# cyberfabric/cyberfabric-core

Hardware: NVIDIA H100
Metric: prompt_bytes_per_sec_bpe_encode (higher is better)
Workload: dtype u32

## Files before the change

### cyberfabric-core_b200/csrc/bpe_kernels.cuh

```cuda
#pragma once
#include <stdint.h>

#include "pretok.cuh"
#include "pretok_fsm.h"
#include "pretok_sync.cuh"
#include "tables.h"
#include "tma.cuh"

namespace cfbpe {

#ifdef CUSIM_EMULATOR
#define CFBPE_DYN_SMEM(name) uint32_t* const name = reinterpret_cast<uint32_t*>(cusim::dyn_smem())
#else
#define CFBPE_DYN_SMEM(name) extern __shared__ __align__(16) uint32_t name[]
#endif

constexpr uint32_t kMaxVocabs = 8;
#ifdef CUSIM_EMULATOR
inline unsigned long long* dbg_counters() { static unsigned long long c[16]; return c; }
#define CFBPE_DBG_COUNT(i) (++dbg_counters()[i])
#else
#define CFBPE_DBG_COUNT(i) ((void)0)
#endif

#ifndef CFBPE_SPLIT_CHUNK
#define CFBPE_SPLIT_CHUNK 64
#endif
constexpr uint32_t kSplitChunk = CFBPE_SPLIT_CHUNK;
constexpr uint32_t kBigPiece = 256;
constexpr uint32_t kScanTileWords = 256;

struct VocabSet {
    TablesView v[kMaxVocabs];
    uint32_t loaded_mask;
};

struct BatchView {
    const uint8_t* bytes;
    const uint64_t* offsets;
    const uint8_t* vocab_ids;
    uint32_t n_prompts;
    uint64_t total_bytes;
};

struct DeviceStatus {
    uint32_t bad_utf8;
    uint32_t n_long;
    uint32_t long_overflow;
    uint32_t long_next;
    uint32_t n_big;
    uint32_t defer_next;
    uint64_t n_tokens;
    uint64_t tok_end;
    unsigned long long long_bytes;
    unsigned long long long_tokens;
    uint32_t miss_n[3];
    uint32_t miss_next[3];
    uint32_t miss_overflow;
    uint32_t extra_n;
    uint32_t split_next;
    uint32_t fix_n;
    uint32_t bad_vocab;
    uint32_t defer_n;
    unsigned long long defer_parts;
};

struct MissLists {
    uint64_t* list[3];
    uint32_t cap[3];
};
__host__ __device__ inline uint32_t miss_class_min_len(uint32_t c) { return c == 0 ? 13u : (c == 1 ? 7u : 1u); }

struct LongPiece { uint64_t start; uint64_t end; uint32_t vocab; uint32_t pad; };

__device__ __forceinline__ uint32_t find_prompt(const uint64_t* __restrict__ offsets, uint32_t n, uint64_t pos) {
    uint32_t lo = 0, hi = n;
    while (hi - lo > 1) {
        const uint32_t mid = (lo + hi) >> 1;
        if (offsets[mid] <= pos) lo = mid; else hi = mid;
    }
    return lo;
}

__device__ __forceinline__ void or_bits(uint32_t* __restrict__ words, uint64_t word, uint32_t bits) {
    if (bits) atomicOr(&words[word], bits);
}

__device__ __forceinline__ void prefetch_l2(const void* p) {
#if !defined(CUSIM_EMULATOR)
    asm volatile("prefetch.global.L2 [%0];" ::"l"(p));
#else
    (void)p;
#endif
}

__device__ __forceinline__ uint64_t same_byte_run_end(const uint8_t* __restrict__ s, uint64_t pos, uint64_t pe, uint32_t c) {
    uint64_t e = pos;
    while (e < pe && (reinterpret_cast<uintptr_t>(s + e) & 15u)) { if (s[e] != c) return e; ++e; }
    const uint32_t w = c * 0x01010101u;
    for (uint64_t a = e; a < pe && a < e + 1024; a += 128) prefetch_l2(s + a);
    while (e + 128 <= pe) {
        if (e + 1024 < pe) prefetch_l2(s + e + 1024);
        uint4 v[8];
#pragma unroll
        for (uint32_t k = 0; k < 8; ++k) v[k] = *reinterpret_cast<const uint4*>(s + e + 16 * k);
        uint32_t d = 0;
#pragma unroll
        for (uint32_t k = 0; k < 8; ++k) d |= (v[k].x ^ w) | (v[k].y ^ w) | (v[k].z ^ w) | (v[k].w ^ w);
        if (d) break;
        e += 128;
    }
    while (e + 16 <= pe) {
        const uint4 v = *reinterpret_cast<const uint4*>(s + e);
        if (v.x != w || v.y != w || v.z != w || v.w != w) break;
        e += 16;
    }
    while (e < pe && s[e] == c) ++e;
    return e;
}
__device__ __forceinline__ bool four_ascii_digits(uint32_t w) {
    const uint32_t t = w ^ 0x30303030u;
    return ((((t & 0x7F7F7F7Fu) + 0x76767676u) | t) & 0x80808080u) == 0u;
}
__device__ __forceinline__ uint64_t ascii_digit_run_end(const uint8_t* __restrict__ s, uint64_t pos, uint64_t pe) {
    uint64_t e = pos;
    while (e < pe && (reinterpret_cast<uintptr_t>(s + e) & 15u)) { if ((s[e] - '0') >= 10u) return e; ++e; }
// ... 322 lines not shown
        sid[bi * 32] = best;
        const uint32_t above2 = alive & ~((2u << bi) - 1u);
        const uint32_t below = alive & ((1u << bi) - 1u);
        const bool wr = above2 != 0, wl = below != 0;
        const uint32_t nn = wr ? static_cast<uint32_t>(__ffs(above2)) - 1u : 0u;
        const uint32_t pv = wl ? 31u - static_cast<uint32_t>(__clz(below)) : 0u;
        uint32_t nr, nl;
        pair_lookup2(T, best, wr ? sid[nn * 32] : 0u, wr, wl ? sid[pv * 32] : 0u, best, wl, nr, nl);
        srk[bi * 32] = nr == kNone ? kNone : ((nr << 5) | bi);
        if (wl) srk[pv * 32] = nl == kNone ? kNone : ((nl << 5) | pv);
    }
    const uint64_t mask = static_cast<uint64_t>(alive) << (pos & 31);
    atomicOr(&tok_bits[pos >> 5], static_cast<uint32_t>(mask));
    if (mask >> 32) atomicOr(&tok_bits[(pos >> 5) + 1], static_cast<uint32_t>(mask >> 32));
    return alive;
}

__device__ __forceinline__ uint32_t kth_set_bit(uint32_t mask, uint32_t k) {
    for (uint32_t i = 0; i < k; ++i) mask &= mask - 1;
    return __ffs(mask) - 1;
}

constexpr uint32_t kPieceMulti = 0x80000000u;
constexpr uint32_t kPieceLong = 0xFFFFFFFEu;
constexpr uint32_t kPieceTileBytes = kPieceWarps * kPieceRange;
static_assert(kPieceTileBytes == 64 * 32, "K3 derives a word's piece tile as word >> 6");
struct DenseIds {
    uint32_t* by_piece;
    uint32_t* extras;
    uint32_t extras_cap;
    uint32_t* tile_pieces;
    uint64_t* piece_base;
};

__global__ void __launch_bounds__(kPieceWarps * 32)
long_scan_kernel(BatchView b, const uint32_t* __restrict__ piece_bits, LongPiece* __restrict__ long_list, uint32_t long_cap,
                 DeviceStatus* status, uint32_t* __restrict__ tile_pieces) {
    const uint32_t lane = threadIdx.x & 31, wic = threadIdx.x >> 5;
    const uint64_t warp = static_cast<uint64_t>(blockIdx.x) * kPieceWarps + wic;
    const uint64_t r0 = warp * kPieceRange;
    const uint64_t r1 = (r0 + kPieceRange < b.total_bytes) ? r0 + kPieceRange : b.total_bytes;
    const bool multi = b.vocab_ids != nullptr;
    const uint64_t base = r0 + 16ull * lane;
    const uint32_t my = (base < b.total_bytes) ? ((piece_bits[base >> 5] >> (16u * (lane & 1u))) & 0xFFFFu) : 0u;
    uint32_t v = my ? (16u * lane + static_cast<uint32_t>(__ffs(my)) - 1u) : 0xFFFFu;
#pragma unroll
    for (uint32_t d = 1; d < 32; d <<= 1) { const uint32_t o = __shfl_down_sync(kFull, v, d); if (lane + d < 32 && o < v) v = o; }
    uint32_t nf_rel = __shfl_down_sync(kFull, v, 1);
    if (lane == 31) nf_rel = 0xFFFFu;
    const bool any_open = __any_sync(kFull, my != 0 && nf_rel == 0xFFFFu);
    uint64_t beyond = b.total_bytes;
    if (any_open) beyond = next_set_bit(piece_bits, r1, b.total_bytes);
    const uint64_t nf = (nf_rel == 0xFFFFu) ? beyond : r0 + nf_rel;
    __shared__ uint32_t s_n[2], s_at[2], s_pieces;
    __shared__ unsigned long long s_bytes;
    if (threadIdx.x < 2) s_n[threadIdx.x] = 0;
    if (threadIdx.x == 0) { s_bytes = 0; s_pieces = 0; }
    __syncthreads();
    const uint32_t np = __reduce_add_sync(kFull, static_cast<uint32_t>(__popc(my)));
    if (lane == 0 && np) atomicAdd(&s_pieces, np);
    bool is_long = false, big = false;
    uint32_t k = 0, pv = 0;
    uint64_t pos = 0;
    if (my && r0 < b.total_bytes) {
        pos = base + (31u - static_cast<uint32_t>(__clz(my)));
        if (nf - pos > 32) {
            is_long = true;
            big = (nf - pos) > kBigPiece;
            pv = multi ? b.vocab_ids[find_prompt(b.offsets, b.n_prompts, pos)] : 0u;
            k = atomicAdd(&s_n[big ? 1 : 0], 1u);
            atomicAdd(&s_bytes, static_cast<unsigned long long>(nf - pos));
        }
    }
    __syncthreads();
    if (threadIdx.x < 2 && s_n[threadIdx.x]) s_at[threadIdx.x] = atomicAdd(threadIdx.x ? &status->n_big : &status->n_long, s_n[threadIdx.x]);
    if (threadIdx.x == 2 && s_bytes) atomicAdd(&status->long_bytes, s_bytes);
    if (threadIdx.x == 3) tile_pieces[blockIdx.x] = s_pieces;
    __syncthreads();
    if (is_long) {
        const uint32_t idx = s_at[big ? 1 : 0] + k;
        if (idx < long_cap) { LongPiece lp; lp.start = pos; lp.end = nf; lp.vocab = pv; lp.pad = 0; long_list[big ? long_cap - 1 - idx : idx] = lp; }
        else atomicOr(&status->long_overflow, 1u);
    }
}

constexpr uint32_t kLookupWarps = 4;
static_assert(kLookupWarps == kPieceWarps, "K2a's CTA is the 2 KiB tile K2s counted");
__global__ void __launch_bounds__(kLookupWarps * 32)
bpe_lookup_kernel(BatchView b, VocabSet vs, const uint32_t* __restrict__ piece_bits, DenseIds dn, MissLists ml, DeviceStatus* status) {
    __shared__ uint16_t s_pos[kLookupWarps][kPieceRange + 2];
    __shared__ uint64_t s_miss0[kLookupWarps * kPieceRange / 13 + 8];
    __shared__ uint64_t s_miss1[kLookupWarps * kPieceRange / 7 + 8];
    __shared__ uint64_t s_miss2[kLookupWarps * kPieceRange / 2 + 8];
    __shared__ uint32_t s_cnt[3], s_base[3], s_nw[kLookupWarps];
    const uint32_t lane = threadIdx.x & 31, wic = threadIdx.x >> 5;
    if (threadIdx.x < 3) s_cnt[threadIdx.x] = 0;
    const uint64_t warp = static_cast<uint64_t>(blockIdx.x) * kLookupWarps + wic;
    const uint64_t r0 = warp * kPieceRange;
    const uint8_t* __restrict__ text = b.bytes;
    const bool multi = b.vocab_ids != nullptr;
    const bool in_range = r0 < b.total_bytes;
    const uint64_t r1 = (r0 + kPieceRange < b.total_bytes) ? r0 + kPieceRange : b.total_bytes;
    uint32_t n_w = 0;
    if (in_range) {
        const uint64_t base = r0 + 16ull * lane;
        const uint32_t my = (base < b.total_bytes) ? ((piece_bits[base >> 5] >> (16u * (lane & 1u))) & 0xFFFFu) : 0u;
        const uint32_t cnt = __popc(my);
        uint32_t incl = cnt;
#pragma unroll
        for (uint32_t d = 1; d < 32; d <<= 1) { const uint32_t o = __shfl_up_sync(kFull, incl, d); if (lane >= d) incl += o; }
        n_w = __shfl_sync(kFull, incl, 31);
        uint32_t slot = incl - cnt;
        for (uint32_t bits = my; bits; bits &= bits - 1) s_pos[wic][slot++] = static_cast<uint16_t>(16u * lane + static_cast<uint32_t>(__ffs(bits)) - 1u);
    }
    if (lane == 0) s_nw[wic] = n_w;
    __syncthreads();
    if (in_range) {
        uint64_t rank0 = dn.piece_base[blockIdx.x];
        for (uint32_t w = 0; w < wic; ++w) rank0 += s_nw[w];
        uint64_t beyond = b.total_bytes;
        if (n_w) beyond = next_set_bit(piece_bits, r1, b.total_bytes);
        TablesView T = vs.v[0];
        uint32_t vid = 0;
        for (uint32_t i = lane; i < n_w; i += 32) {
            const uint32_t off = s_pos[wic][i];
            const uint64_t pos = r0 + off;
            const uint64_t end = (i + 1 < n_w) ? r0 + s_pos[wic][i + 1] : beyond;
            if (end - pos > 32) { dn.by_piece[rank0 + i] = kPieceLong; continue; }
            const uint32_t len = static_cast<uint32_t>(end - pos);
            if (multi) {
                const uint32_t pv = b.vocab_ids[find_prompt(b.offsets, b.n_prompts, pos)];
                if (pv != vid) { vid = pv; T = vs.v[vid]; }
            }
            const uint32_t tok = (len == 1) ? T.byte2id[text[pos]] : whole_piece_lookup(T, text + pos, len);
            if (tok != kNone) {
// ... 39 lines not shown
    for (uint32_t c = 0; c < 3; ++c) {
        const uint32_t n = status->miss_n[c];
        const uint64_t* __restrict__ list = ml.list[c];
        for (;;) {
            uint32_t t0 = 0;
            if (lane == 0) t0 = atomicAdd(&status->miss_next[c], 32u);
            t0 = __shfl_sync(kFull, t0, 0);
            if (t0 >= n) break;
            const uint32_t i = t0 + lane;
            uint32_t alive = 0, rank = 0;
            if (i < n) {
                const uint64_t e = list[i];
                const uint64_t pos = e & 0xFFFFFFFFull;
                rank = static_cast<uint32_t>(e >> 32);
                const uint64_t end = next_set_bit(piece_bits, pos + 1, b.total_bytes);
                if (multi) {
                    const uint32_t pv = b.vocab_ids[find_prompt(b.offsets, b.n_prompts, pos)];
                    if (pv != vid) { vid = pv; T = vs.v[vid]; }
                }
                alive = merge_piece_in_lane(T, text, pos, static_cast<uint32_t>(end - pos), sid, srk, tok_bits);
            }
            const uint32_t cnt = __popc(alive);
            uint32_t incl = cnt;
#pragma unroll
            for (uint32_t d = 1; d < 32; d <<= 1) { const uint32_t o = __shfl_up_sync(kFull, incl, d); if (lane >= d) incl += o; }
            const uint32_t total = __shfl_sync(kFull, incl, 31);
            uint32_t base = 0;
            if (lane == 0 && total) base = atomicAdd(&status->extra_n, total);
            base = __shfl_sync(kFull, base, 0);
            if (cnt) {
                uint32_t slot = base + incl - cnt;
                if (slot + cnt <= dn.extras_cap) {
                    dn.by_piece[rank] = kPieceMulti | slot;
                    for (uint32_t bits = alive; bits; bits &= bits - 1) dn.extras[slot++] = sid[(static_cast<uint32_t>(__ffs(bits)) - 1u) * 32];
                } else atomicOr(&status->miss_overflow, 1u);
            }
            __syncwarp();
        }
    }
}

struct LongScratch {
    uint32_t* rank;
    uint32_t* aux0;
    uint32_t* aux1;
};

__device__ __forceinline__ uint32_t warp_min_u32(uint32_t v) {
#pragma unroll
    for (uint32_t d = 16; d; d >>= 1) { const uint32_t o = __shfl_xor_sync(kFull, v, d); v = o < v ? o : v; }
    return v;
}

__device__ __forceinline__ bool select_chunk(uint32_t r, uint32_t rmin, uint32_t lane, uint32_t& carry, uint32_t& sel_ballot) {
    const bool cand = (r == rmin);
    const uint32_t C = __ballot_sync(kFull, cand);
    const uint32_t z = ~C & lanemask_lt(lane);
    const uint32_t s = z ? (32u - __clz(z)) : 0u;
    const uint32_t cnt = lane - s + (s == 0 ? carry : 0u);
    const bool sel = cand && !(cnt & 1u);
    sel_ballot = __ballot_sync(kFull, sel);
    const uint32_t nz = ~C;
    carry = nz ? static_cast<uint32_t>(__clz(nz)) : (carry + 32u);
    return sel;
}

__device__ __forceinline__ void array_round(const TablesView& T, uint32_t* id, uint32_t* rk, uint32_t* a0, uint32_t* a1,
                                            uint32_t m, uint32_t rmin, uint32_t lane) {
    uint32_t carry = 0, prevS = 0, cut = kNone;
    for (uint32_t base = 0; base < m && cut == kNone; base += 32) {
        const uint32_t i = base + lane;
        const uint32_t r = (i + 1 < m) ? rk[i] : kNone;
        uint32_t S;
        const bool sel = select_chunk(r, rmin, lane, carry, S);
        bool viol = false;
        if (sel) {
            const bool selm2 = (lane >= 2) ? ((S >> (lane - 2)) & 1u) : ((prevS >> (30 + lane)) & 1u);
            uint32_t L = kNone, R = kNone;
            if (i > 0) L = pair_lookup(T, selm2 ? rmin : id[i - 1], rmin);
            if (i + 2 < m) R = pair_lookup(T, rmin, id[i + 2]);
            a0[i] = L;
            a1[i] = R;
            viol = (L < rmin) || (R < rmin);
        }
        const uint32_t V = __ballot_sync(kFull, viol);
        if (V) cut = base + (__ffs(V) - 1);
        prevS = S;
    }
    __syncwarp();
    carry = 0; prevS = 0;
    for (uint32_t base = 0; base < m && base <= cut; base += 32) {
        const uint32_t i = base + lane;
        const uint32_t r = (i + 1 < m) ? rk[i] : kNone;
        uint32_t S;
        const bool sel = select_chunk(r, rmin, lane, carry, S);
        const bool app = sel && i <= cut;
        const bool selm2 = (lane >= 2) ? ((S >> (lane - 2)) & 1u) : ((prevS >> (30 + lane)) & 1u);
        uint32_t L = kNone;
        if (app) {
            L = a0[i];
            id[i] = rmin;
            id[i + 1] = kNone;
            rk[i] = a1[i];
        }
        __syncwarp();
        if (app && i > 0) rk[selm2 ? i - 2 : i - 1] = L;
        __syncwarp();
        prevS = S;
    }
}
template <uint32_t kPosBits>
__device__ __forceinline__ uint32_t array_compact(uint32_t* id, uint32_t* rk, uint32_t m, uint32_t lane, uint32_t& rmin_out) {
    uint32_t out = 0, nmin = kNone;
    for (uint32_t base = 0; base < m; base += 32) {
        const uint32_t i = base + lane;
        const uint32_t myid = (i < m) ? id[i] : kNone;
        uint32_t myrk = (i < m) ? rk[i] : kNone;
        if (kPosBits && myrk != kNone) myrk >>= kPosBits;
        const bool keep = myid != kNone;
        const uint32_t K = __ballot_sync(kFull, keep);
        const uint32_t pos = out + __popc(K & lanemask_lt(lane));
        __syncwarp();
        if (keep) { id[pos] = myid; rk[pos] = myrk; nmin = myrk < nmin ? myrk : nmin; }
        out += __popc(K);
    }
    __syncwarp();
    rmin_out = warp_min_u32(nmin);
    return out;
}

constexpr uint32_t kListMax = 65535;
constexpr uint32_t kMedSmem = 256;

__device__ __forceinline__ bool key_less(uint32_t r1, uint32_t p1, uint32_t r2, uint32_t p2) { return r1 < r2 || (r1 == r2 && p1 < p2); }

__device__ __forceinline__ void list_rounds_multi(const TablesView& T, uint32_t* id, uint32_t* rk, uint32_t* link, uint32_t* nid,
                                                  uint32_t m, uint32_t lane) {
    constexpr uint32_t kNoPrev = 0xFFFFu;
    for (uint32_t i = lane; i < m; i += 32) {
        link[i] = ((i + 1) << 16) | (i ? i - 1 : kNoPrev);
        nid[i] = (i + 1 < m) ? id[i + 1] : kNone;
    }
    __syncwarp();
    const uint32_t c = ((m + 31) / 32) | 1u;
    const uint32_t lo = lane * c < m ? lane * c : m;
    const uint32_t hi = lo + c < m ? lo + c : m;
    for (;;) {
        uint32_t m1 = kNone, p1 = 0, m2 = kNone, p2 = 0;
        for (uint32_t xb = lo; xb < hi; xb += 16) {
            uint32_t v[16];
#pragma unroll
            for (uint32_t t = 0; t < 16; ++t) v[t] = (xb + t < hi) ? rk[xb + t] : kNone;
#pragma unroll
            for (uint32_t t = 0; t < 16; ++t) {
                if (v[t] < m1) { m2 = m1; p2 = p1; m1 = v[t]; p1 = xb + t; }
                else if (v[t] < m2) { m2 = v[t]; p2 = xb + t; }
            }
        }
        if (!__any_sync(kFull, m1 != kNone)) break;
        const bool valid = m1 != kNone;
        const uint32_t x = p1, r = m1;
        uint32_t j = 0, q = kNoPrev, k = m, L = kNone, R = kNone;
        if (valid) {
            const uint32_t li = link[x];
            j = li >> 16; q = li & 0xFFFFu;
            k = link[j] >> 16;
            const uint32_t idk = nid[j];
            const uint32_t idq = (q != kNoPrev) ? id[q] : 0u;
            pair_lookup2(T, r, idk, k < m, idq, r, q != kNoPrev, R, L);
        }
        uint32_t c_r = m2, c_p = p2;
        if (key_less(L, q, c_r, c_p)) { c_r = L; c_p = q; }
        if (key_less(R, x, c_r, c_p)) { c_r = R; c_p = x; }
        const uint32_t xq = x | (q << 16), jk = j | (k << 16);
        bool pending = valid, accepted = false;
        uint32_t bound_r = kNone, bound_p = 0xFFFFFFFFu;
        for (;;) {
            const uint32_t best = __reduce_min_sync(kFull, pending ? ((r << 5) | lane) : kNone);
            if (best == kNone) break;
            const uint32_t s = best & 31u, br = best >> 5;
            const uint32_t sxq = __shfl_sync(kFull, xq, s), sjk = __shfl_sync(kFull, jk, s);
            const uint32_t bp = sxq & 0xFFFFu, sq = sxq >> 16, sj = sjk & 0xFFFFu, sk = sjk >> 16;
            if (!key_less(br, bp, bound_r, bound_p)) break;
            const uint32_t gone_here = (accepted && (j == bp || x == sj)) ? 1u : 0u;
            const uint32_t near_here = (accepted && (x == sq || x == bp || x == sj || x == sk || j == sq || j == bp || j == sj || j == sk ||
                                                     q == bp || q == sj || k == bp || k == sj)) ? 2u : 0u;
            const uint32_t flags = __reduce_or_sync(kFull, gone_here | near_here);
            const bool gone = flags & 1u;
            if (!gone && (flags & 2u)) break;
            if (lane == s) { pending = false; accepted = !gone; }
            const uint32_t sr = __shfl_sync(kFull, gone ? m2 : c_r, s), sp = __shfl_sync(kFull, gone ? p2 : c_p, s);
            if (key_less(sr, sp, bound_r, bound_p)) { bound_r = sr; bound_p = sp; }
        }
        if (accepted) {
            id[x] = r; id[j] = kNone; rk[j] = kNone; rk[x] = R;
            link[x] = (k << 16) | q;
            nid[x] = nid[j];
            if (k < m) link[k] = (link[k] & 0xFFFF0000u) | x;
            if (q != kNoPrev) { rk[q] = L; nid[q] = r; }
        }
        __syncwarp();
    }
}

constexpr uint32_t kNoKey = 0xFFFFFFFFu;
template <uint32_t kWarps, uint32_t kPosBits>
__device__ __forceinline__ bool list_rounds_par(const TablesView& T, uint32_t* id, uint32_t* kk, uint32_t* link, uint32_t* claim,
                                                uint32_t m, uint32_t* s_red, uint32_t* dirty = nullptr) {
    constexpr uint32_t kNoPrev = 0xFFFFu, kPosMask = (1u << kPosBits) - 1u, P = kWarps * 32;
    const uint32_t tid = threadIdx.x % P, lane = tid & 31, wid = tid >> 5;
    auto group_sync = [&]() { if (kWarps == 1) __syncwarp(); else __syncthreads(); };
    for (uint32_t i = tid; i < m; i += P) {
        const uint32_t r = kk[i];
        kk[i] = (r == kNone) ? kNoKey : ((r << kPosBits) | i);
        link[i] = ((i + 1) << 16) | (i ? i - 1 : kNoPrev);
        claim[i] = kNoKey;
    }
    if (dirty) dirty[tid] = 0;
    uint32_t* const eq_flag = s_red + 2 * kWarps;
    if (kWarps > 1 && tid == 0) { eq_flag[0] = 0; eq_flag[1] = 0; }
    group_sync();
    uint32_t eq_run = 0;
    uint32_t c = (m + P - 1) / P;
    if (c > 1) c |= 1u;
    const uint32_t lo = tid * c < m ? tid * c : m;
    const uint32_t hi = lo + c < m ? lo + c : m;
    const uint32_t inv_c = (1u << 20) / c + 1u;
    bool have = false;
    uint32_t m1 = kNoKey, m2 = kNoKey, j = 0, q = kNoPrev, k = m, Lk = kNoKey, Rk = kNoKey;
    for (uint32_t round = 0;; ++round) {
        if (dirty && have && dirty[tid]) have = false;
        if (!have) {
            if (dirty) dirty[tid] = 0;
            m1 = kNoKey; m2 = kNoKey;
            uint32_t n1 = kNoKey, n2 = kNoKey;
            uint32_t xb = lo;
            for (; xb + 8 <= hi; xb += 8) {
                uint32_t v[8];
#pragma unroll
                for (uint32_t t = 0; t < 8; ++t) v[t] = kk[xb + t];
#pragma unroll
                for (uint32_t t = 0; t < 8; t += 2) {
                    const uint32_t a = v[t], b = v[t + 1];
                    const uint32_t ha = a > m1 ? a : m1, hb = b > n1 ? b : n1;
                    m2 = ha < m2 ? ha : m2; n2 = hb < n2 ? hb : n2;
                    m1 = a < m1 ? a : m1; n1 = b < n1 ? b : n1;
                }
            }
            if (xb < hi) {
                uint32_t v[8];
#pragma unroll
                for (uint32_t t = 0; t < 8; ++t) v[t] = (xb + t < hi) ? kk[xb + t] : kNoKey;
#pragma unroll
                for (uint32_t t = 0; t < 8; t += 2) {
                    const uint32_t a = v[t], b = v[t + 1];
                    const uint32_t ha = a > m1 ? a : m1, hb = b > n1 ? b : n1;
                    m2 = ha < m2 ? ha : m2; n2 = hb < n2 ? hb : n2;
                    m1 = a < m1 ? a : m1; n1 = b < n1 ? b : n1;
                }
            }
            {
                const uint32_t lo1 = m1 < n1 ? m1 : n1, hi1 = m1 < n1 ? n1 : m1;
                const uint32_t s2 = m2 < n2 ? m2 : n2;
                m1 = lo1; m2 = hi1 < s2 ? hi1 : s2;
            }
            Lk = kNoKey; Rk = kNoKey;
            if (m1 != kNoKey) {
                const uint32_t x = m1 & kPosMask, r = m1 >> kPosBits;
                const uint32_t li = link[x];
                j = li >> 16; q = li & 0xFFFFu;
                k = link[j] >> 16;
                const uint32_t idk = (k < m) ? id[k] : 0u;
                const uint32_t idq = (q != kNoPrev) ? id[q] : 0u;
                uint32_t R, L;
                pair_lookup2(T, r, idk, k < m, idq, r, q != kNoPrev, R, L);
                if (R != kNone) Rk = (R << kPosBits) | x;
                if (L != kNone) Lk = (L << kPosBits) | q;
            }
            have = dirty != nullptr;
        }
        const bool valid = m1 != kNoKey;
        const uint32_t x = m1 & kPosMask, r = m1 >> kPosBits;
        uint32_t v = kNoKey;
        bool viol = false;
        if (valid) {
            uint32_t cc = m2 < Lk ? m2 : Lk;
            cc = cc < Rk ? cc : Rk;
            viol = cc <= m1;
            v = cc > m1 + 1u ? cc : m1 + 1u;
            if (v == kNoKey) v = kNoKey - 1u;
            atomicMin(&claim[x], m1);
            atomicMin(&claim[j], m1);
        }
        group_sync();
        if (kWarps > 1 && tid == 0) eq_flag[(round + 1u) & 1u] = 0;
        if (valid) {
            uint32_t lowest = claim[x];
            const uint32_t cj = claim[j];
            lowest = cj < lowest ? cj : lowest;
            if (q != kNoPrev) { const uint32_t cq = claim[q]; lowest = cq < lowest ? cq : lowest; }
            if (k < m) { const uint32_t ck = claim[k]; lowest = ck < lowest ? ck : lowest; }
            if (lowest < m1) { v = m1; have = false; }
        }
        uint32_t cut = __reduce_min_sync(kFull, v);
        if (kWarps > 1) {
            uint32_t* red = s_red + (round & 1u) * kWarps;
            if (lane == 0) red[wid] = cut;
            __syncthreads();
            cut = red[0];
#pragma unroll
            for (uint32_t w = 1; w < kWarps; ++w) { const uint32_t o = red[w]; cut = o < cut ? o : cut; }
        } else {
            __syncwarp();
        }
        if (cut == kNoKey) return true;
        if (kWarps > 1 && tid == 0) CFBPE_DBG_COUNT(6);
        if (kWarps > 1 && valid && m1 < cut) CFBPE_DBG_COUNT(7);
        bool eq = valid && m1 < cut && !viol && (cut >> kPosBits) == (m1 >> kPosBits);
        if (kWarps == 1) eq = __any_sync(kFull, eq);
        else if (eq) eq_flag[round & 1u] = 1u;
        if (valid) {
            claim[x] = kNoKey; claim[j] = kNoKey;
            if (m1 < cut) {
                id[x] = r; id[j] = kNone;
                kk[j] = kNoKey; kk[x] = Rk;
                link[x] = (k << 16) | q;
                if (k < m) link[k] = (link[k] & 0xFFFF0000u) | x;
                if (q != kNoPrev) kk[q] = Lk;
                have = false;
                if (dirty) {
                    if (j >= hi) dirty[(j * inv_c) >> 20] = 1u;
                    if (q != kNoPrev && q < lo) dirty[(q * inv_c) >> 20] = 1u;
                }
            }
        }
        group_sync();
        if (kWarps > 1) eq = eq_flag[round & 1u] != 0u;
        eq_run = eq ? eq_run + 1u : 0u;
        if (eq_run >= 3u) {
            const uint32_t er = cut >> kPosBits;
            uint32_t cnt = 0;
            for (uint32_t y = lo; y < hi; ++y) cnt += (kk[y] >> kPosBits) == er ? 1u : 0u;
            cnt = __reduce_add_sync(kFull, cnt);
            if (kWarps > 1) {
                uint32_t* sum = s_red + 2 * kWarps + 2;
                if (lane == 0) sum[wid] = cnt;
                __syncthreads();
                cnt = 0;
#pragma unroll
                for (uint32_t w = 0; w < kWarps; ++w) cnt += sum[w];
                __syncthreads();
            }
            if (cnt >= 8u && cnt * 32u >= m) return false;
            eq_run = 0;
        }
    }
}

__device__ __forceinline__ void flag_parts(const uint32_t* id, uint32_t* copy_to, uint32_t m, uint64_t start,
                                           uint32_t* __restrict__ tok_bits, DeviceStatus* status, uint32_t lane) {
    for (uint32_t base = 0; base < m; base += 32) {
        const uint32_t i = base + lane;
        const uint32_t v = (i < m) ? id[i] : kNone;
        const bool alive = v != kNone;
        if (alive && copy_to) copy_to[i] = v;
        const uint32_t A = __ballot_sync(kFull, alive);
        if (lane == 0 && A) {
            atomicAdd(&status->long_tokens, static_cast<unsigned long long>(__popc(A)));
            const uint64_t pos = start + base;
            const uint32_t sh = static_cast<uint32_t>(pos & 31);
            atomicOr(&tok_bits[pos >> 5], A << sh);
            if (sh && (A >> (32 - sh))) atomicOr(&tok_bits[(pos >> 5) + 1], A >> (32 - sh));
        }
    }
}

constexpr uint32_t kDeferMaxParts = 4096;
constexpr uint32_t kListSmemBytes = kDeferMaxParts * 16;
constexpr uint32_t kListMaxRank = (1u << 20) - 1u;
__device__ __forceinline__ bool list_kernel_takes(const TablesView& T, uint32_t n_bytes) { return n_bytes <= kDeferMaxParts && T.n_ranks < kListMaxRank; }


constexpr uint32_t kLongWarps = 4;
#ifndef CFBPE_LONG_MIN_CTAS
#define CFBPE_LONG_MIN_CTAS (32 / kLongWarps)
#endif
__global__ void __launch_bounds__(kLongWarps * 32, CFBPE_LONG_MIN_CTAS)
bpe_long_kernel(BatchView b, VocabSet vs, LongPiece* long_list, DeviceStatus* status,
                uint32_t long_cap, uint32_t* __restrict__ ids_by_pos, LongScratch sc, uint32_t* __restrict__ tok_bits) {
    __shared__ uint32_t s_med[kLongWarps][4][kMedSmem];
    const uint32_t lane = threadIdx.x & 31;
    const uint32_t n_big = status->n_big;
    const uint32_t n_all = status->long_overflow ? 0u : status->n_long + n_big;
    for (;;) {
        uint32_t item = 0;
        if (lane == 0) item = atomicAdd(&status->long_next, 1u);
        item = __shfl_sync(kFull, item, 0);
        if (item >= n_all) break;
        const uint32_t slot = item < n_big ? long_cap - 1 - item : item - n_big;
        const LongPiece lp = long_list[slot];
        const TablesView T = vs.v[lp.vocab];
        const uint8_t* __restrict__ p = b.bytes + lp.start;
        const uint32_t n = static_cast<uint32_t>(lp.end - lp.start);
#ifndef CFBPE_NO_DEFER
        if (item < n_big && list_kernel_takes(T, n)) continue;
#endif
        uint32_t* const gid = ids_by_pos + lp.start;
        const bool in_smem = n <= kMedSmem;
        uint32_t* id = in_smem ? s_med[threadIdx.x >> 5][0] : gid;
        uint32_t* rk = in_smem ? s_med[threadIdx.x >> 5][1] : sc.rank + lp.start;
        uint32_t* a0 = in_smem ? s_med[threadIdx.x >> 5][2] : sc.aux0 + lp.start;
        uint32_t* a1 = in_smem ? s_med[threadIdx.x >> 5][3] : sc.aux1 + lp.start;

        if (n <= T.max_token_len) {
            uint32_t t = kNone;
            if (lane == 0) t = piece_lookup(T, p, n);
            t = __shfl_sync(kFull, t, 0);
            if (t != kNone) {
                if (lane == 0) { gid[0] = t; atomicOr(&tok_bits[lp.start >> 5], 1u << (lp.start & 31)); atomicAdd(&status->long_tokens, 1ull); }
                continue;
            }
        }
        uint32_t m = n;
        uint32_t rmin = kNone;
        for (uint32_t i = lane; i < n; i += 32) {
            const uint32_t c0 = p[i];
            id[i] = T.byte2id[c0];
            const uint32_t r = (i + 1 < n) ? T.bytepair[(c0 << 8) | p[i + 1]] : kNone;
            rk[i] = r;
            rmin = r < rmin ? r : rmin;
        }
        rmin = warp_min_u32(rmin);
        __syncwarp();

        bool deferred = false;
        while (rmin != kNone) {
            array_round(T, id, rk, a0, a1, m, rmin, lane);
            const uint32_t before = m;
            m = array_compact<0>(id, rk, m, lane, rmin);
            const uint32_t merged = before - m;
            if (rmin == kNone || merged * 8u >= m || m <= 32u || m > kListMax) continue;
            if (in_smem) {
                if (list_rounds_par<1, 8>(T, id, rk, a0, a1, m, nullptr)) break;
                if (lane == 0) CFBPE_DBG_COUNT(1);
                m = array_compact<8>(id, rk, m, lane, rmin);
                continue;
            }
            if (lane == 0) CFBPE_DBG_COUNT(5);
            list_rounds_multi(T, id, rk, a0, a1, m, lane);
            __syncwarp();
            break;
        }
        if (deferred) continue;
        __syncwarp();
        flag_parts(id, in_smem ? gid : nullptr, m, lp.start, tok_bits, status, lane);
        __syncwarp();
    }
}

constexpr uint32_t kCtaChunk = 16;

__device__ __forceinline__ void cta_array_round(const TablesView& T, uint32_t* id, uint32_t* rk, uint32_t* a0, uint32_t* a1,
                                                uint32_t m, uint32_t rmin, uint32_t* s_scan, uint32_t* s_sel) {
    const uint32_t P = blockDim.x, t = threadIdx.x;
    const uint32_t c = (m + P - 1) / P;
    const uint32_t lo = t * c < m ? t * c : m, hi = lo + c < m ? lo + c : m;
    uint32_t tail = 0, all = 1;
    for (uint32_t i = lo; i < hi; ++i) {
        const bool cand = (i + 1 < m) && rk[i] == rmin;
        if (cand) ++tail; else { tail = 0; all = 0; }
    }
    s_scan[t] = (all << 31) | tail;
    if (t == 0) s_scan[P] = kNone;
    for (uint32_t w = t; w < kDeferMaxParts / 32; w += P) s_sel[w] = 0;
    __syncthreads();
    uint32_t cnt = 0;
    for (uint32_t u = t; u > 0 && lo < m;) {
        const uint32_t e = s_scan[--u];
        cnt += e & 0x7FFFFFFFu;
        if (!(e >> 31)) break;
    }
    uint32_t sel_bits = 0;
    for (uint32_t i = lo; i < hi; ++i) {
        const bool cand = (i + 1 < m) && rk[i] == rmin;
        if (cand && !(cnt & 1u)) { sel_bits |= 1u << (i - lo); atomicOr(&s_sel[i >> 5], 1u << (i & 31)); }
        cnt = cand ? cnt + 1 : 0;
    }
    __syncthreads();
    uint32_t m2_bits = 0;
    for (uint32_t bts = sel_bits; bts; bts &= bts - 1) {
        const uint32_t k = static_cast<uint32_t>(__ffs(bts)) - 1u, i = lo + k;
        const bool selm2 = i >= 2 && ((s_sel[(i - 2) >> 5] >> ((i - 2) & 31)) & 1u);
        uint32_t L = kNone, R = kNone;
        if (i > 0) L = pair_lookup(T, selm2 ? rmin : id[i - 1], rmin);
        if (i + 2 < m) R = pair_lookup(T, rmin, id[i + 2]);
        a0[i] = L; a1[i] = R;
        if (selm2) m2_bits |= 1u << k;
        if (L < rmin || R < rmin) atomicMin(&s_scan[P], i);
    }
    __syncthreads();
    const uint32_t cut = s_scan[P];
    for (uint32_t bts = sel_bits; bts; bts &= bts - 1) {
        const uint32_t i = lo + static_cast<uint32_t>(__ffs(bts)) - 1u;
        if (i > cut) break;
        id[i] = rmin; id[i + 1] = kNone; rk[i] = a1[i];
    }
    __syncthreads();
    for (uint32_t bts = sel_bits; bts; bts &= bts - 1) {
        const uint32_t k = static_cast<uint32_t>(__ffs(bts)) - 1u, i = lo + k;
// ... 348 lines not shown
```

Measured before the change: 35.81 billion.

## Bin long pieces by length and process short ones with half-warp lane groups

The long-piece scan now sorts medium pieces into three length bins (33-64, 65-128, 129-256 bytes), stored as packed 64-bit entries, while big pieces keep the full struct at the tail of the list. The long kernel hands out tickets per bin, and the shortest bin is processed by 16-lane groups so each warp merges two pieces at once instead of leaving half its lanes idle. The warp primitives (ballot, min, sum, compaction, list rounds) are templated on group size to make this possible. In exchange, divergence handling becomes more complex, there are extra any_sync loops, and the list layout changes, which could lead to capacity or overflow mismatches if host-side sizing does not match.

```diff
diff --git a/cyberfabric-core_b200/csrc/bpe_kernels.cuh b/cyberfabric-core_b200/csrc/bpe_kernels.cuh
--- a/cyberfabric-core_b200/csrc/bpe_kernels.cuh
+++ b/cyberfabric-core_b200/csrc/bpe_kernels.cuh
@@ -46,6 +46,7 @@
 struct DeviceStatus {
     uint32_t bad_utf8;
     uint32_t n_long;
+    uint32_t n_bin[3];
     uint32_t long_overflow;
     uint32_t long_next;
     uint32_t n_big;
@@ -72,6 +73,18 @@
 __host__ __device__ inline uint32_t miss_class_min_len(uint32_t c) { return c == 0 ? 13u : (c == 1 ? 7u : 1u); }
 
 struct LongPiece { uint64_t start; uint64_t end; uint32_t vocab; uint32_t pad; };
+
+constexpr uint32_t kLongBins = 3;
+__host__ __device__ inline uint32_t long_bin_of(uint64_t len) { return len <= 64 ? 0u : (len <= 128 ? 1u : 2u); }
+__host__ __device__ inline uint64_t long_bin_cap(uint32_t c, uint64_t total) { return total / ((32u << c) + 1u) + 1u; }
+__host__ __device__ inline uint64_t long_bin_base(uint32_t c, uint64_t total) {
+    uint64_t s = 0;
+    for (uint32_t k = 0; k < c; ++k) s += long_bin_cap(k, total);
+    return s;
+}
+__host__ __device__ inline uint64_t pack_medium(uint64_t start, uint64_t len, uint32_t vocab) {
+    return start | ((len - 33u) << 48) | (static_cast<uint64_t>(vocab) << 56);
+}
 
 __device__ __forceinline__ uint32_t find_prompt(const uint64_t* __restrict__ offsets, uint32_t n, uint64_t pos) {
     uint32_t lo = 0, hi = n;
@@ -500,35 +513,51 @@
     uint64_t beyond = b.total_bytes;
     if (any_open) beyond = next_set_bit(piece_bits, r1, b.total_bytes);
     const uint64_t nf = (nf_rel == 0xFFFFu) ? beyond : r0 + nf_rel;
-    __shared__ uint32_t s_n[2], s_at[2], s_pieces;
+    __shared__ uint32_t s_n[kLongBins + 1], s_at[kLongBins + 1], s_pieces;
     __shared__ unsigned long long s_bytes;
-    if (threadIdx.x < 2) s_n[threadIdx.x] = 0;
-    if (threadIdx.x == 0) { s_bytes = 0; s_pieces = 0; }
+    __shared__ uint64_t s_first[kLongBins], s_cap[kLongBins + 1];
+    if (threadIdx.x <= kLongBins) s_n[threadIdx.x] = 0;
+    if (threadIdx.x == 0) {
+        s_bytes = 0; s_pieces = 0;
+        uint64_t at = 0;
+        for (uint32_t c = 0; c < kLongBins; ++c) { s_first[c] = at; s_cap[c] = long_bin_cap(c, b.total_bytes); at += s_cap[c]; }
+        const uint64_t bin_entries = (at + 2) / 3;
+        s_cap[kLongBins] = long_cap > bin_entries ? long_cap - bin_entries : 0u;
+    }
     __syncthreads();
     const uint32_t np = __reduce_add_sync(kFull, static_cast<uint32_t>(__popc(my)));
     if (lane == 0 && np) atomicAdd(&s_pieces, np);
-    bool is_long = false, big = false;
-    uint32_t k = 0, pv = 0;
+    bool is_long = false;
+    uint32_t k = 0, pv = 0, cls = 0;
     uint64_t pos = 0;
     if (my && r0 < b.total_bytes) {
         pos = base + (31u - static_cast<uint32_t>(__clz(my)));
         if (nf - pos > 32) {
             is_long = true;
-            big = (nf - pos) > kBigPiece;
+            cls = (nf - pos) > kBigPiece ? kLongBins : long_bin_of(nf - pos);
             pv = multi ? b.vocab_ids[find_prompt(b.offsets, b.n_prompts, pos)] : 0u;
-            k = atomicAdd(&s_n[big ? 1 : 0], 1u);
+            k = atomicAdd(&s_n[cls], 1u);
             atomicAdd(&s_bytes, static_cast<unsigned long long>(nf - pos));
         }
     }
     __syncthreads();
-    if (threadIdx.x < 2 && s_n[threadIdx.x]) s_at[threadIdx.x] = atomicAdd(threadIdx.x ? &status->n_big : &status->n_long, s_n[threadIdx.x]);
-    if (threadIdx.x == 2 && s_bytes) atomicAdd(&status->long_bytes, s_bytes);
-    if (threadIdx.x == 3) tile_pieces[blockIdx.x] = s_pieces;
+    if (threadIdx.x <= kLongBins && s_n[threadIdx.x])
+        s_at[threadIdx.x] = atomicAdd(threadIdx.x < kLongBins ? &status->n_bin[threadIdx.x] : &status->n_big, s_n[threadIdx.x]);
+    if (threadIdx.x == kLongBins + 1 && s_bytes) atomicAdd(&status->long_bytes, s_bytes);
+    if (threadIdx.x == kLongBins + 2) tile_pieces[blockIdx.x] = s_pieces;
     __syncthreads();
     if (is_long) {
-        const uint32_t idx = s_at[big ? 1 : 0] + k;
-        if (idx < long_cap) { LongPiece lp; lp.start = pos; lp.end = nf; lp.vocab = pv; lp.pad = 0; long_list[big ? long_cap - 1 - idx : idx] = lp; }
-        else atomicOr(&status->long_overflow, 1u);
+        const uint32_t idx = s_at[cls] + k;
+        if (idx < s_cap[cls]) {
+            if (cls < kLongBins) {
+                reinterpret_cast<uint64_t*>(long_list)[s_first[cls] + idx] = pack_medium(pos, nf - pos, pv);
+            } else {
+                LongPiece lp; lp.start = pos; lp.end = nf; lp.vocab = pv; lp.pad = 0;
+                long_list[long_cap - 1 - idx] = lp;
+            }
+        } else {
+            atomicOr(&status->long_overflow, 1u);
+        }
     }
 }
 
@@ -674,30 +703,64 @@
     return v;
 }
 
+template <uint32_t G>
+__device__ __forceinline__ uint32_t group_ballot(bool p) {
+    const uint32_t B = __ballot_sync(kFull, p);
+    if constexpr (G == 32) return B;
+    else return (B >> ((threadIdx.x & 31u) & ~(G - 1u))) & ((1u << G) - 1u);
+}
+template <uint32_t G>
+__device__ __forceinline__ bool loop_any(bool p) {
+    if constexpr (G == 32) return p;
+    else return __any_sync(kFull, p);
+}
+template <uint32_t G>
+__device__ __forceinline__ bool group_any(bool p) {
+    if constexpr (G == 32) return __any_sync(kFull, p);
+    else return group_ballot<G>(p) != 0u;
+}
+template <uint32_t G>
+__device__ __forceinline__ uint32_t group_min(uint32_t v) {
+#pragma unroll
+    for (uint32_t d = G / 2; d; d >>= 1) { const uint32_t o = __shfl_xor_sync(kFull, v, d); v = o < v ? o : v; }
+    return v;
+}
+template <uint32_t G>
+__device__ __forceinline__ uint32_t group_sum(uint32_t v) {
+    if constexpr (G == 32) return __reduce_add_sync(kFull, v);
+#pragma unroll
+    for (uint32_t d = G / 2; d; d >>= 1) v += __shfl_xor_sync(kFull, v, d);
+    return v;
+}
+
+template <uint32_t G>
 __device__ __forceinline__ bool select_chunk(uint32_t r, uint32_t rmin, uint32_t lane, uint32_t& carry, uint32_t& sel_ballot) {
+    const uint32_t gl = lane & (G - 1u);
     const bool cand = (r == rmin);
-    const uint32_t C = __ballot_sync(kFull, cand);
-    const uint32_t z = ~C & lanemask_lt(lane);
+    const uint32_t C = group_ballot<G>(cand);
+    const uint32_t z = ~C & lanemask_lt(gl);
     const uint32_t s = z ? (32u - __clz(z)) : 0u;
-    const uint32_t cnt = lane - s + (s == 0 ? carry : 0u);
+    const uint32_t cnt = gl - s + (s == 0 ? carry : 0u);
     const bool sel = cand && !(cnt & 1u);
-    sel_ballot = __ballot_sync(kFull, sel);
-    const uint32_t nz = ~C;
-    carry = nz ? static_cast<uint32_t>(__clz(nz)) : (carry + 32u);
+    sel_ballot = group_ballot<G>(sel);
+    const uint32_t nz = G == 32 ? ~C : (~C & ((1u << (G & 31u)) - 1u));
+    carry = nz ? static_cast<uint32_t>(__clz(nz)) - (32u - G) : (carry + G);
     return sel;
 }
 
+template <uint32_t G>
 __device__ __forceinline__ void array_round(const TablesView& T, uint32_t* id, uint32_t* rk, uint32_t* a0, uint32_t* a1,
                                             uint32_t m, uint32_t rmin, uint32_t lane) {
+    const uint32_t gl = lane & (G - 1u);
     uint32_t carry = 0, prevS = 0, cut = kNone;
-    for (uint32_t base = 0; base < m && cut == kNone; base += 32) {
-        const uint32_t i = base + lane;
-        const uint32_t r = (i + 1 < m) ? rk[i] : kNone;
+    for (uint32_t base = 0; loop_any<G>(base < m && cut == kNone); base += G) {
+        const uint32_t i = base + gl;
+        const uint32_t r = ((G == 32 || cut == kNone) && i + 1 < m) ? rk[i] : kNone;
         uint32_t S;
-        const bool sel = select_chunk(r, rmin, lane, carry, S);
+        const bool sel = select_chunk<G>(r, rmin, lane, carry, S);
         bool viol = false;
         if (sel) {
-            const bool selm2 = (lane >= 2) ? ((S >> (lane - 2)) & 1u) : ((prevS >> (30 + lane)) & 1u);
+            const bool selm2 = (gl >= 2) ? ((S >> (gl - 2)) & 1u) : ((prevS >> (G - 2 + gl)) & 1u);
             uint32_t L = kNone, R = kNone;
             if (i > 0) L = pair_lookup(T, selm2 ? rmin : id[i - 1], rmin);
             if (i + 2 < m) R = pair_lookup(T, rmin, id[i + 2]);
@@ -705,19 +768,19 @@
             a1[i] = R;
             viol = (L < rmin) || (R < rmin);
         }
-        const uint32_t V = __ballot_sync(kFull, viol);
+        const uint32_t V = group_ballot<G>(viol);
         if (V) cut = base + (__ffs(V) - 1);
         prevS = S;
     }
     __syncwarp();
     carry = 0; prevS = 0;
-    for (uint32_t base = 0; base < m && base <= cut; base += 32) {
-        const uint32_t i = base + lane;
-        const uint32_t r = (i + 1 < m) ? rk[i] : kNone;
+    for (uint32_t base = 0; loop_any<G>(base < m && base <= cut); base += G) {
+        const uint32_t i = base + gl;
+        const uint32_t r = ((G == 32 || base <= cut) && i + 1 < m) ? rk[i] : kNone;
         uint32_t S;
-        const bool sel = select_chunk(r, rmin, lane, carry, S);
+        const bool sel = select_chunk<G>(r, rmin, lane, carry, S);
         const bool app = sel && i <= cut;
-        const bool selm2 = (lane >= 2) ? ((S >> (lane - 2)) & 1u) : ((prevS >> (30 + lane)) & 1u);
+        const bool selm2 = (gl >= 2) ? ((S >> (gl - 2)) & 1u) : ((prevS >> (G - 2 + gl)) & 1u);
         uint32_t L = kNone;
         if (app) {
             L = a0[i];
@@ -731,23 +794,24 @@
         prevS = S;
     }
 }
-template <uint32_t kPosBits>
+template <uint32_t kPosBits, uint32_t G>
 __device__ __forceinline__ uint32_t array_compact(uint32_t* id, uint32_t* rk, uint32_t m, uint32_t lane, uint32_t& rmin_out) {
+    const uint32_t gl = lane & (G - 1u);
     uint32_t out = 0, nmin = kNone;
-    for (uint32_t base = 0; base < m; base += 32) {
-        const uint32_t i = base + lane;
+    for (uint32_t base = 0; loop_any<G>(base < m); base += G) {
+        const uint32_t i = base + gl;
         const uint32_t myid = (i < m) ? id[i] : kNone;
         uint32_t myrk = (i < m) ? rk[i] : kNone;
         if (kPosBits && myrk != kNone) myrk >>= kPosBits;
         const bool keep = myid != kNone;
-        const uint32_t K = __ballot_sync(kFull, keep);
-        const uint32_t pos = out + __popc(K & lanemask_lt(lane));
+        const uint32_t K = group_ballot<G>(keep);
+        const uint32_t pos = out + __popc(K & lanemask_lt(gl));
         __syncwarp();
         if (keep) { id[pos] = myid; rk[pos] = myrk; nmin = myrk < nmin ? myrk : nmin; }
         out += __popc(K);
     }
     __syncwarp();
-    rmin_out = warp_min_u32(nmin);
+    rmin_out = group_min<G>(nmin);
     return out;
 }
 
@@ -826,12 +890,15 @@
 }
 
 constexpr uint32_t kNoKey = 0xFFFFFFFFu;
-template <uint32_t kWarps, uint32_t kPosBits>
+template <uint32_t kWarps, uint32_t kPosBits, uint32_t G = 32>
 __device__ __forceinline__ bool list_rounds_par(const TablesView& T, uint32_t* id, uint32_t* kk, uint32_t* link, uint32_t* claim,
                                                 uint32_t m, uint32_t* s_red, uint32_t* dirty = nullptr) {
-    constexpr uint32_t kNoPrev = 0xFFFFu, kPosMask = (1u << kPosBits) - 1u, P = kWarps * 32;
+    static_assert(kWarps == 1 || G == 32, "lane groups are parts of one warp");
+    constexpr uint32_t kNoPrev = 0xFFFFu, kPosMask = (1u << kPosBits) - 1u, P = kWarps == 1 ? G : kWarps * 32;
+    constexpr bool kOneGroup = P >= 32;
     const uint32_t tid = threadIdx.x % P, lane = tid & 31, wid = tid >> 5;
     auto group_sync = [&]() { if (kWarps == 1) __syncwarp(); else __syncthreads(); };
+    bool live = true, res = true;
     for (uint32_t i = tid; i < m; i += P) {
         const uint32_t r = kk[i];
         kk[i] = (r == kNone) ? kNoKey : ((r << kPosBits) | i);
@@ -843,7 +910,7 @@
     if (kWarps > 1 && tid == 0) { eq_flag[0] = 0; eq_flag[1] = 0; }
     group_sync();
     uint32_t eq_run = 0;
-    uint32_t c = (m + P - 1) / P;
+    uint32_t c = m > P ? (m + P - 1) / P : 1u;
     if (c > 1) c |= 1u;
     const uint32_t lo = tid * c < m ? tid * c : m;
     const uint32_t hi = lo + c < m ? lo + c : m;
@@ -886,6 +953,7 @@
                 const uint32_t s2 = m2 < n2 ? m2 : n2;
                 m1 = lo1; m2 = hi1 < s2 ? hi1 : s2;
             }
+            if (!kOneGroup && !live) m1 = kNoKey;
             Lk = kNoKey; Rk = kNoKey;
             if (m1 != kNoKey) {
                 const uint32_t x = m1 & kPosMask, r = m1 >> kPosBits;
@@ -924,7 +992,7 @@
             if (k < m) { const uint32_t ck = claim[k]; lowest = ck < lowest ? ck : lowest; }
             if (lowest < m1) { v = m1; have = false; }
         }
-        uint32_t cut = __reduce_min_sync(kFull, v);
+        uint32_t cut = kOneGroup ? __reduce_min_sync(kFull, v) : group_min<G>(v);
         if (kWarps > 1) {
             uint32_t* red = s_red + (round & 1u) * kWarps;
             if (lane == 0) red[wid] = cut;
@@ -935,11 +1003,14 @@
         } else {
             __syncwarp();
         }
-        if (cut == kNoKey) return true;
+        if (cut == kNoKey) {
+            if constexpr (kOneGroup) return true;
+            if (live) { live = false; res = true; }
+        }
         if (kWarps > 1 && tid == 0) CFBPE_DBG_COUNT(6);
         if (kWarps > 1 && valid && m1 < cut) CFBPE_DBG_COUNT(7);
         bool eq = valid && m1 < cut && !viol && (cut >> kPosBits) == (m1 >> kPosBits);
-        if (kWarps == 1) eq = __any_sync(kFull, eq);
+        if (kWarps == 1) eq = group_any<G>(eq);
         else if (eq) eq_flag[round & 1u] = 1u;
         if (valid) {
             claim[x] = kNoKey; claim[j] = kNoKey;
@@ -959,11 +1030,12 @@
         group_sync();
         if (kWarps > 1) eq = eq_flag[round & 1u] != 0u;
         eq_run = eq ? eq_run + 1u : 0u;
-        if (eq_run >= 3u) {
+        if (loop_any<kOneGroup ? 32 : G>(eq_run >= 3u)) {
+            const bool ask = eq_run >= 3u;
             const uint32_t er = cut >> kPosBits;
             uint32_t cnt = 0;
-            for (uint32_t y = lo; y < hi; ++y) cnt += (kk[y] >> kPosBits) == er ? 1u : 0u;
-            cnt = __reduce_add_sync(kFull, cnt);
+            if (ask) for (uint32_t y = lo; y < hi; ++y) cnt += (kk[y] >> kPosBits) == er ? 1u : 0u;
+            cnt = kOneGroup ? __reduce_add_sync(kFull, cnt) : group_sum<G>(cnt);
             if (kWarps > 1) {
                 uint32_t* sum = s_red + 2 * kWarps + 2;
                 if (lane == 0) sum[wid] = cnt;
@@ -973,21 +1045,30 @@
                 for (uint32_t w = 0; w < kWarps; ++w) cnt += sum[w];
                 __syncthreads();
             }
-            if (cnt >= 8u && cnt * 32u >= m) return false;
-            eq_run = 0;
-        }
-    }
-}
-
+            if (ask) {
+                if (cnt >= 8u && cnt * 32u >= m) {
+                    if constexpr (kOneGroup) return false;
+                    live = false; res = false;
+                }
+                eq_run = 0;
+            }
+        }
+        if constexpr (!kOneGroup) {
+            if (!__any_sync(kFull, live)) return res;
+        }
+    }
+}
+
+template <uint32_t G = 32>
 __device__ __forceinline__ void flag_parts(const uint32_t* id, uint32_t* copy_to, uint32_t m, uint64_t start,
                                            uint32_t* __restrict__ tok_bits, DeviceStatus* status, uint32_t lane) {
-    for (uint32_t base = 0; base < m; base += 32) {
-        const uint32_t i = base + lane;
+    for (uint32_t base = 0; loop_any<G>(base < m); base += G) {
+        const uint32_t i = base + (lane & (G - 1u));
         const uint32_t v = (i < m) ? id[i] : kNone;
         const bool alive = v != kNone;
         if (alive && copy_to) copy_to[i] = v;
-        const uint32_t A = __ballot_sync(kFull, alive);
-        if (lane == 0 && A) {
+        const uint32_t A = group_ballot<G>(alive);
+        if ((lane & (G - 1u)) == 0 && A) {
             atomicAdd(&status->long_tokens, static_cast<unsigned long long>(__popc(A)));
             const uint64_t pos = start + base;
             const uint32_t sh = static_cast<uint32_t>(pos & 31);
@@ -1002,6 +1083,116 @@
 constexpr uint32_t kListMaxRank = (1u << 20) - 1u;
 __device__ __forceinline__ bool list_kernel_takes(const TablesView& T, uint32_t n_bytes) { return n_bytes <= kDeferMaxParts && T.n_ranks < kListMaxRank; }
 
+
+template <uint32_t G>
+__device__ __forceinline__ void long_group_ticket(const BatchView& b, const VocabSet& vs, const uint64_t* __restrict__ bin, uint32_t n_bin,
+                                                  uint32_t first, uint32_t (*s)[kMedSmem], uint32_t* __restrict__ ids_by_pos,
+                                                  uint32_t* __restrict__ tok_bits, DeviceStatus* status) {
+    const uint32_t lane = threadIdx.x & 31, gb = lane & ~(G - 1u), gl = lane & (G - 1u);
+    const uint32_t item = first + gb / G;
+    LongPiece lp = {0, 0, 0, 0};
+    if (item < n_bin) {
+        const uint64_t e = bin[item];
+        lp.start = e & ((1ull << 48) - 1u);
+        lp.end = lp.start + ((e >> 48) & 0xFFu) + 33u;
+        lp.vocab = static_cast<uint32_t>(e >> 56);
+    }
+    const TablesView T = vs.v[lp.vocab];
+    const uint8_t* __restrict__ p = b.bytes + lp.start;
+    const uint32_t n = static_cast<uint32_t>(lp.end - lp.start);
+    uint32_t* const gid = ids_by_pos + lp.start;
+    uint32_t* const id = s[0] + 8 * gb;
+    uint32_t* const rk = s[1] + 8 * gb;
+    uint32_t* const a0 = s[2] + 8 * gb;
+    uint32_t* const a1 = s[3] + 8 * gb;
+
+    uint32_t t = kNone;
+    if (gl == 0 && n && n <= T.max_token_len) t = piece_lookup(T, p, n);
+    t = __shfl_sync(kFull, t, gb);
+    if (t != kNone && gl == 0) { gid[0] = t; atomicOr(&tok_bits[lp.start >> 5], 1u << (lp.start & 31)); atomicAdd(&status->long_tokens, 1ull); }
+    uint32_t m = t == kNone ? n : 0u;
+    uint32_t rmin = kNone;
+    for (uint32_t i = gl; i < m; i += G) {
+        const uint32_t c0 = p[i];
+        id[i] = T.byte2id[c0];
+        const uint32_t r = (i + 1 < m) ? T.bytepair[(c0 << 8) | p[i + 1]] : kNone;
+        rk[i] = r;
+        rmin = r < rmin ? r : rmin;
+    }
+    rmin = group_min<G>(rmin);
+    __syncwarp();
+
+    while (loop_any<G>(rmin != kNone)) {
+        const bool on = rmin != kNone;
+        array_round<G>(T, id, rk, a0, a1, on ? m : 0u, on ? rmin : 0u, lane);
+        uint32_t r2;
+        const uint32_t m2 = array_compact<0, G>(id, rk, on ? m : 0u, lane, r2);
+        bool list = false;
+        if (on) {
+            const uint32_t merged = m - m2;
+            m = m2; rmin = r2;
+            list = !(rmin == kNone || merged * 8u >= m || m <= G);
+        }
+        if (!loop_any<G>(list)) continue;
+        const bool done = list_rounds_par<1, 8, G>(T, id, rk, a0, a1, list ? m : 0u, nullptr);
+        if (list && !done && gl == 0) CFBPE_DBG_COUNT(1);
+        const uint32_t m3 = array_compact<8, G>(id, rk, list && !done ? m : 0u, lane, r2);
+        if (list) {
+            if (done) rmin = kNone;
+            else { m = m3; rmin = r2; }
+        }
+    }
+    __syncwarp();
+    flag_parts<G>(id, gid, m, lp.start, tok_bits, status, lane);
+    __syncwarp();
+}
+
+__device__ __forceinline__ void long_giant(const TablesView& T, const LongPiece& lp, const BatchView& b, uint32_t* __restrict__ ids_by_pos,
+                                           const LongScratch& sc, uint32_t* __restrict__ tok_bits, DeviceStatus* status) {
+    const uint32_t lane = threadIdx.x & 31;
+    const uint8_t* __restrict__ p = b.bytes + lp.start;
+    const uint32_t n = static_cast<uint32_t>(lp.end - lp.start);
+    uint32_t* const id = ids_by_pos + lp.start;
+    uint32_t* const rk = sc.rank + lp.start;
+    uint32_t* const a0 = sc.aux0 + lp.start;
+    uint32_t* const a1 = sc.aux1 + lp.start;
+
+    if (n <= T.max_token_len) {
+        uint32_t t = kNone;
+        if (lane == 0) t = piece_lookup(T, p, n);
+        t = __shfl_sync(kFull, t, 0);
+        if (t != kNone) {
+            if (lane == 0) { id[0] = t; atomicOr(&tok_bits[lp.start >> 5], 1u << (lp.start & 31)); atomicAdd(&status->long_tokens, 1ull); }
+            return;
+        }
+    }
+    uint32_t m = n;
+    uint32_t rmin = kNone;
+    for (uint32_t i = lane; i < n; i += 32) {
+        const uint32_t c0 = p[i];
+        id[i] = T.byte2id[c0];
+        const uint32_t r = (i + 1 < n) ? T.bytepair[(c0 << 8) | p[i + 1]] : kNone;
+        rk[i] = r;
+        rmin = r < rmin ? r : rmin;
+    }
+    rmin = warp_min_u32(rmin);
+    __syncwarp();
+
+    while (rmin != kNone) {
+        array_round<32>(T, id, rk, a0, a1, m, rmin, lane);
+        const uint32_t before = m;
+        m = array_compact<0, 32>(id, rk, m, lane, rmin);
+        const uint32_t merged = before - m;
+        if (rmin == kNone || merged * 8u >= m || m <= 32u || m > kListMax) continue;
+        if (lane == 0) CFBPE_DBG_COUNT(5);
+        list_rounds_multi(T, id, rk, a0, a1, m, lane);
+        __syncwarp();
+        break;
+    }
+    __syncwarp();
+    flag_parts(id, nullptr, m, lp.start, tok_bits, status, lane);
+    __syncwarp();
+}
 
 constexpr uint32_t kLongWarps = 4;
 #ifndef CFBPE_LONG_MIN_CTAS
@@ -1011,72 +1202,34 @@
 bpe_long_kernel(BatchView b, VocabSet vs, LongPiece* long_list, DeviceStatus* status,
                 uint32_t long_cap, uint32_t* __restrict__ ids_by_pos, LongScratch sc, uint32_t* __restrict__ tok_bits) {
     __shared__ uint32_t s_med[kLongWarps][4][kMedSmem];
+    __shared__ const uint64_t* s_bin[kLongBins];
+    if (threadIdx.x < kLongBins) s_bin[threadIdx.x] = reinterpret_cast<const uint64_t*>(long_list) + long_bin_base(threadIdx.x, b.total_bytes);
+    __syncthreads();
     const uint32_t lane = threadIdx.x & 31;
     const uint32_t n_big = status->n_big;
-    const uint32_t n_all = status->long_overflow ? 0u : status->n_long + n_big;
+    const uint32_t n0 = status->n_bin[0], n1 = status->n_bin[1], n2 = status->n_bin[2];
+    if (blockIdx.x == 0 && threadIdx.x == 0) status->n_long = n0 + n1 + n2;
+    const uint32_t t2 = n_big + n2, t1 = t2 + n1, n_all = status->long_overflow ? 0u : t1 + (n0 + 1) / 2;
     for (;;) {
         uint32_t item = 0;
         if (lane == 0) item = atomicAdd(&status->long_next, 1u);
         item = __shfl_sync(kFull, item, 0);
         if (item >= n_all) break;
-        const uint32_t slot = item < n_big ? long_cap - 1 - item : item - n_big;
-        const LongPiece lp = long_list[slot];
-        const TablesView T = vs.v[lp.vocab];
-        const uint8_t* __restrict__ p = b.bytes + lp.start;
-        const uint32_t n = static_cast<uint32_t>(lp.end - lp.start);
+        uint32_t (*const s)[kMedSmem] = s_med[threadIdx.x >> 5];
+        if (item >= t1) {
+            long_group_ticket<16>(b, vs, s_bin[0], n0, 2 * (item - t1), s, ids_by_pos, tok_bits, status);
+        } else if (item >= t2) {
+            long_group_ticket<32>(b, vs, s_bin[1], n1, item - t2, s, ids_by_pos, tok_bits, status);
+        } else if (item >= n_big) {
+            long_group_ticket<32>(b, vs, s_bin[2], n2, item - n_big, s, ids_by_pos, tok_bits, status);
+        } else {
+            const LongPiece lp = long_list[long_cap - 1 - item];
+            const TablesView T = vs.v[lp.vocab];
 #ifndef CFBPE_NO_DEFER
-        if (item < n_big && list_kernel_takes(T, n)) continue;
+            if (list_kernel_takes(T, static_cast<uint32_t>(lp.end - lp.start))) continue;
 #endif
-        uint32_t* const gid = ids_by_pos + lp.start;
-        const bool in_smem = n <= kMedSmem;
-        uint32_t* id = in_smem ? s_med[threadIdx.x >> 5][0] : gid;
-        uint32_t* rk = in_smem ? s_med[threadIdx.x >> 5][1] : sc.rank + lp.start;
-        uint32_t* a0 = in_smem ? s_med[threadIdx.x >> 5][2] : sc.aux0 + lp.start;
-        uint32_t* a1 = in_smem ? s_med[threadIdx.x >> 5][3] : sc.aux1 + lp.start;
-
-        if (n <= T.max_token_len) {
-            uint32_t t = kNone;
-            if (lane == 0) t = piece_lookup(T, p, n);
-            t = __shfl_sync(kFull, t, 0);
-            if (t != kNone) {
-                if (lane == 0) { gid[0] = t; atomicOr(&tok_bits[lp.start >> 5], 1u << (lp.start & 31)); atomicAdd(&status->long_tokens, 1ull); }
-                continue;
-            }
-        }
-        uint32_t m = n;
-        uint32_t rmin = kNone;
-        for (uint32_t i = lane; i < n; i += 32) {
-            const uint32_t c0 = p[i];
-            id[i] = T.byte2id[c0];
-            const uint32_t r = (i + 1 < n) ? T.bytepair[(c0 << 8) | p[i + 1]] : kNone;
-            rk[i] = r;
-            rmin = r < rmin ? r : rmin;
-        }
-        rmin = warp_min_u32(rmin);
-        __syncwarp();
-
-        bool deferred = false;
-        while (rmin != kNone) {
-            array_round(T, id, rk, a0, a1, m, rmin, lane);
-            const uint32_t before = m;
-            m = array_compact<0>(id, rk, m, lane, rmin);
-            const uint32_t merged = before - m;
-            if (rmin == kNone || merged * 8u >= m || m <= 32u || m > kListMax) continue;
-            if (in_smem) {
-                if (list_rounds_par<1, 8>(T, id, rk, a0, a1, m, nullptr)) break;
-                if (lane == 0) CFBPE_DBG_COUNT(1);
-                m = array_compact<8>(id, rk, m, lane, rmin);
-                continue;
-            }
-            if (lane == 0) CFBPE_DBG_COUNT(5);
-            list_rounds_multi(T, id, rk, a0, a1, m, lane);
-            __syncwarp();
-            break;
-        }
-        if (deferred) continue;
-        __syncwarp();
-        flag_parts(id, in_smem ? gid : nullptr, m, lp.start, tok_bits, status, lane);
-        __syncwarp();
+            long_giant(T, lp, b, ids_by_pos, sc, tok_bits, status);
+        }
     }
 }
 
```

After: 36.42 billion (median of 6 runs). 1.7% higher.
